# MundyRepo/MuNDy

Measured on AMD Instinct MI355X. Metric: timesteps/sec, 10^6 spherocylinders, frictionless LCP contact (BBPGD), higher is better.
Workload: dtype f64; 1 GPU; configs[2]: 1M spherocylinders r=0.5 L=2 at 40% volume fraction, random packing, AABB+0.1 neighbour list, frictionless LCP tol 1e-05; bodies_per_gpu=1000000, bodies_total=1000000, contacts_per_gpu=7621833, contacts_total=7621833, parallelism=single GPU (N > 1: the same system, hilbert domain decomposition with RCCL halo)

## Files before the change

mundy_amd/csrc/convex.hip:

```cpp
#include <cstdlib>
#include <memory>
#include <mutex>
#include <type_traits>
#include <vector>

#include "../../include/mundy_hip_contact_force.h"
#include "../../include/mundy_hip_hydro_solve.h"
#include "mhip_internal.hpp"

namespace mhip {

constexpr unsigned kProfileStride = 8;
constexpr double kSmallStep = 1e-6;
constexpr double kBBEps = 1e-15 * 10;
constexpr double kLowest = -1.7976931348623157e308;

#ifndef MHIP_STREAM_UNROLL
#define MHIP_STREAM_UNROLL 4
#endif
#ifndef MHIP_STREAM_GRID
#define MHIP_STREAM_GRID 1048576
#endif
constexpr int kStreamUnroll = MHIP_STREAM_UNROLL;
__device__ inline size_t stream_first() { return blockIdx.x * (size_t)(kBlock * kStreamUnroll) + threadIdx.x; }
// ... 314 lines not shown
  const unsigned g = stream_grid(vec ? (n + 1) / 2 : n);
  if (vec) k_copy<true><<<g, kBlock, 0, s>>>(n, dst, src);
  else k_copy<false><<<g, kBlock, 0, s>>>(n, dst, src);
  MHIP_LAUNCH_CHECK();
  return MHIP_SUCCESS;
}

#ifndef MHIP_NT
#define MHIP_NT 3
#endif
typedef double mhip_d2v __attribute__((ext_vector_type(2)));
typedef int mhip_i2v __attribute__((ext_vector_type(2)));
template <bool NT> __device__ inline double ld_s(const double* p) { return NT ? __builtin_nontemporal_load(p) : *p; }
template <bool NT> __device__ inline int32_t ld_s(const int32_t* p) { return NT ? __builtin_nontemporal_load(p) : *p; }
template <bool NT> __device__ inline double2 ld_s(const double2* p) {
  if (!NT) return *p;
  const mhip_d2v v = __builtin_nontemporal_load(reinterpret_cast<const mhip_d2v*>(p));
  return make_double2(v.x, v.y);
}
template <bool NT> __device__ inline int2 ld_s(const int2* p) {
  if (!NT) return *p;
  const mhip_i2v v = __builtin_nontemporal_load(reinterpret_cast<const mhip_i2v*>(p));
  return make_int2(v.x, v.y);
}
template <bool NT> __device__ inline V3 ld_s3(const double* p, size_t i) {
  return {ld_s<NT>(p + 3 * i), ld_s<NT>(p + 3 * i + 1), ld_s<NT>(p + 3 * i + 2)};
}

struct SolverState {
  double step, residual, num, den;
  unsigned iter;
  unsigned flips;
  int converged, done, converged_at_init;
};

enum XMode { X_APPLY = 0, X_INIT = 1, X_SOLVE = 2 };
enum Kinematics { KIN_TRANS = 0, KIN_RIGID = 1, KIN_ROD = 2 };

struct OpView {
  size_t C, N;
  const int2* pairs;
  const double *normal, *ra, *rb, *mt, *mr;
  const int32_t *inc_ptr, *inc;
  const double* half;
  double* vel;
  double dt;
  size_t body_first, body_count;
  const unsigned char* counted;
  const double *arc_s, *arc_t;
  const double* axis;
  double* omega;
  int xcd_aware;
  size_t c_first, c_end;
  unsigned part_offset, part_stride;
  unsigned long long* body_mask;
  const unsigned char* pos;
  const int32_t* aptr;
  const int32_t* aent;
  const double* arec;
  size_t arec_stride;
  const unsigned long long* snap_mask;
  double* vel_alt;
  double* drift;
  const double* arm_max;
  const double* fire_at;
  int32_t* fired;
  unsigned long long* tier_counters;
  double* force_rows;
};

__device__ inline size_t xcd_tile(size_t lin, size_t ntiles, unsigned T) {
  if (T == 0) return lin;
  const size_t W = 8 * (size_t)T;
  const size_t g = lin / W, r = lin % W;
  if ((g + 1) * W > ntiles) return lin;
  return g * W + (r % 8) * T + r / 8;
}

template <int MODE, bool PACKED, bool NT = false>
__device__ inline double2 iterate_load(size_t c, const double* __restrict__ xt, const double* __restrict__ gt) {
  if (MODE == X_SOLVE) {
    if (PACKED) return ld_s<NT>(reinterpret_cast<const double2*>(xt) + c);
    return make_double2(xt[c], gt[c]);
  }
  return make_double2(xt[c], 0.0);
}
template <int MODE>
__device__ inline double iterate_value(double2 p, double step, bool step_is_zero, const Space& sp) {
  if (MODE == X_SOLVE) {
    const double v = step_is_zero ? 1.0 * p.x : 1.0 * p.x + (-step) * p.y;
    return sp.project(v);
  }
  return p.x;
}
// ... 15 lines not shown
#ifndef MHIP_KBODY_FLAT
#define MHIP_KBODY_FLAT 2
#endif
#ifndef MHIP_KBODY_EARLY_FROM
#define MHIP_KBODY_EARLY_FROM 3
#endif
#ifndef MHIP_KBODY_FLAT3_ABOVE
#define MHIP_KBODY_FLAT3_ABOVE 0.9
#endif
template <int MODE, int KIN, int G, int U, bool PACKED, int TRACK = 0, int FLATP = 0>
__global__ void __launch_bounds__(kBlock, MHIP_KBODY_WAVES)
    k_body(OpView op, const SolverState* __restrict__ st, const double* __restrict__ X0, const double* __restrict__ X1,
           const double* __restrict__ G0, const double* __restrict__ G1, Space sp) {
  constexpr bool FLAT = FLATP > 0 && MODE == X_SOLVE && PACKED;
  constexpr bool kRegTrack = TRACK == 2 && MODE == X_SOLVE && PACKED;
  constexpr int kFlatPlanes = kRegTrack ? ((KIN == KIN_RIGID) ? 4 : 3) : ((KIN == KIN_RIGID) ? 3 : 2);
  __shared__ double2 flat_img[FLAT ? kFlatPlanes * FLATP * kBlock : 1];
  const size_t tile = xcd_tile(blockIdx.x, gridDim.x, op.xcd_aware);
  const size_t t = tile * (size_t)blockDim.x + threadIdx.x;
  const int sub = static_cast<int>(t % G);
  const bool has_body = t / G < op.body_count;
  if (!FLAT && !has_body) return;
  const size_t b = op.body_first + (has_body ? t / G : op.body_count - 1);
  int32_t E0 = 0, E1 = 0;
  if constexpr (FLAT) {
    if (op.aptr != nullptr) {
      const size_t tb0r = tile * (size_t)(kBlock / G);
      const size_t tb0 = (tb0r < op.body_count) ? tb0r : op.body_count;
      const size_t tb1 = (tb0 + kBlock / G < op.body_count) ? tb0 + kBlock / G : op.body_count;
      E0 = op.aptr[op.body_first + tb0];
      E1 = op.aptr[op.body_first + tb1];
    }
  }
  const double* xt = X0;
  const double* gt = G0;
  double step = 0.0;
  double* vel_new = op.vel;
  if (MODE == X_SOLVE) {
    const int done = st->done;
    const bool odd = st->flips & 1u;
    step = st->step;
    if (done) return;
    if (odd) {
      xt = X1;
      gt = G1;
    }
    if (op.vel_alt) vel_new = odd ? op.vel : op.vel_alt;
  }
  const bool step_is_zero = fabs(-step) < kZeroTol;
  constexpr int HW = (KIN == KIN_RIGID) ? 6 : (KIN == KIN_ROD ? 4 : 3);
  DD3 Fdd{{0.0, 0.0}, {0.0, 0.0}, {0.0, 0.0}}, Tdd{{0.0, 0.0}, {0.0, 0.0}, {0.0, 0.0}};
  const int32_t beg = op.inc_ptr[b], end = op.inc_ptr[b + 1];
  double mt = 0.0, mr = 0.0;
  V3 axis{0.0, 0.0, 0.0};
  constexpr bool track = TRACK != 0 && MODE == X_SOLVE && PACKED;
  constexpr bool track_regs = kRegTrack;
  constexpr bool track_rows = track && !track_regs;
  V3 dF{0.0, 0.0, 0.0}, dS{0.0, 0.0, 0.0};
  constexpr bool kEarlyTail = FLAT && FLATP >= MHIP_KBODY_EARLY_FROM && track;
  constexpr bool kEarlySnap = FLAT && FLATP >= MHIP_KBODY_EARLY_FROM;
  double drift_old = 0.0, fire_thr = 0.0;
  unsigned long long snap_early = 0ull;
  if (kEarlySnap) {
    const unsigned long long* src = (op.aptr != nullptr && op.body_mask != nullptr)
                                        ? op.snap_mask
                                        : reinterpret_cast<const unsigned long long*>(op.vel);
    snap_early = src[b];
  }
  unsigned long long mask_early = 0ull;
  if (kEarlySnap) {
    const unsigned long long* src = (op.body_mask != nullptr) ? op.body_mask
                                                              : reinterpret_cast<const unsigned long long*>(op.vel);
    mask_early = src[b];
  }
  double2 o0 = make_double2(0.0, 0.0), o1 = o0, o2 = o0;
  if (sub == 0) {
    mt = op.mt[b];
    if (KIN != KIN_TRANS) mr = op.mr[b];
    if (KIN == KIN_ROD) axis = load3(op.axis, b);
    if (kEarlyTail) {
      drift_old = op.drift[b];
      if (op.fire_at != nullptr) fire_thr = op.fire_at[b];
      if (track_rows) {
        const double* vel_old = op.vel_alt ? ((vel_new == op.vel) ? op.vel_alt : op.vel) : op.vel;
        const double2* vo = reinterpret_cast<const double2*>(vel_old + 6 * b);
        o0 = vo[0];
        o1 = vo[1];
        o2 = vo[2];
      }
    }
  }
  auto process = [&](const int32_t* __restrict__ ent, const double* __restrict__ rec, const int32_t* kk,
                     const bool eager, const size_t planes = 0) {
    int32_t e[U];
    double lam[U], xo[U];
    double2 h0[U], h1[U], h2[U];
    auto fetch = [&](int u) {
      const size_t k = static_cast<size_t>(kk[u]);
      if (planes != 0) {
        const double2* H2 = reinterpret_cast<const double2*>(rec) + k;
        h0[u] = H2[0];
        h1[u] = H2[planes];
        if (KIN == KIN_RIGID) h2[u] = H2[2 * planes];
      } else if (KIN == KIN_TRANS) {
        const double* H = rec + k * HW;
        h0[u] = make_double2(H[0], H[1]);
        h1[u] = make_double2(H[2], 0.0);
      } else {
        const double2* H2 = reinterpret_cast<const double2*>(rec + k * HW);
        h0[u] = H2[0];
        h1[u] = H2[1];
// ... 9 lines not shown
    double2 pit[U];
#pragma unroll
    for (int u = 0; u < U; ++u)
      pit[u] = iterate_load<MODE, PACKED>(e[u] >= 0 ? static_cast<size_t>(e[u] >> 1) : 0, xt, gt);
#pragma unroll
    for (int u = 0; u < U; ++u) {
      xo[u] = (track_regs && e[u] >= 0) ? pit[u].x : 0.0;
      lam[u] = (e[u] >= 0) ? iterate_value<MODE>(pit[u], step, step_is_zero, sp) : 0.0;
    }
    if (!eager) {
#pragma unroll
      for (int u = 0; u < U; ++u)
        if (lam[u] != 0.0 || (track_regs && xo[u] != 0.0)) fetch(u);
    }
#pragma unroll
    for (int u = 0; u < U; ++u) {
      if (lam[u] == 0.0 && !(track_regs && xo[u] != 0.0)) continue;
      const V3 n{h0[u].x, h0[u].y, h1[u].x};
      if (track_regs) {
        const double dl = (e[u] & 1) ? lam[u] - xo[u] : xo[u] - lam[u];
        const V3 df{dl * n.x, dl * n.y, dl * n.z};
        dF = dF + df;
        if (KIN == KIN_ROD) dS = dS + h1[u].y * df;
        if (KIN == KIN_RIGID) dS = dS + cross(V3{h1[u].y, h2[u].x, h2[u].y}, df);
      }
      if (lam[u] == 0.0) continue;
      V3 f{lam[u] * n.x, lam[u] * n.y, lam[u] * n.z};
      if (!(e[u] & 1)) f = V3{-f.x, -f.y, -f.z};
      dd_add(Fdd, f);
      if (KIN == KIN_RIGID) dd_add(Tdd, cross(V3{h1[u].y, h2[u].x, h2[u].y}, f));
      if (KIN == KIN_ROD) dd_add(Tdd, h1[u].y * f);
    }
  };
  const bool masked = PACKED && MODE == X_SOLVE && op.body_mask != nullptr && sp.kind == MHIP_SPACE_LOWER_BOUND &&
                      sp.lo == 0.0 && step >= 0.0 && step <= 1.7976931348623157e308;
  int32_t full_from = beg;
  if (masked) {
    if (op.aptr != nullptr) {
      const int32_t ab = op.aptr[b], ae = op.aptr[b + 1];
      if constexpr (FLAT) {
        constexpr int kChunk = FLATP * kBlock;
        constexpr bool NTS = (MHIP_NT & 1) != 0;
        double2* const pl0 = flat_img;
        double2* const pl1 = flat_img + kChunk;
        double2* const pl2 = flat_img + (kFlatPlanes - 1) * kChunk;
        for (int32_t base = E0; base < E1; base += kChunk) {
          int32_t fe[FLATP];
          double2 r0[FLATP], r1[FLATP], r2[FLATP];
          bool live[FLATP];
#pragma unroll
          for (int p = 0; p < FLATP; ++p) {
            const int32_t k = base + p * kBlock + static_cast<int32_t>(threadIdx.x);
            live[p] = k < E1;
            fe[p] = ld_s<NTS>(op.aent + (live[p] ? k : E1 - 1));
          }
#pragma unroll
          for (int p = 0; p < FLATP; ++p) {
            const int32_t k0 = base + p * kBlock + static_cast<int32_t>(threadIdx.x);
            const size_t k = static_cast<size_t>(live[p] ? k0 : E1 - 1);
            r2[p] = make_double2(0.0, 0.0);
            const double2* H2 = reinterpret_cast<const double2*>(op.arec) + k;
            r0[p] = ld_s<NTS>(H2);
            r1[p] = ld_s<NTS>(H2 + op.arec_stride);
            if (KIN == KIN_RIGID) r2[p] = ld_s<NTS>(H2 + 2 * op.arec_stride);
          }
#pragma unroll
          for (int p = 0; p < FLATP; ++p)
            if (!live[p]) fe[p] = -1;
          double2 pit[FLATP];
#pragma unroll
// ... 41 lines not shown
                if (a3.y != 0.0) {
                  const V3 df{a3.y * n.x, a3.y * n.y, a3.y * n.z};
                  dF = dF + df;
                  if (KIN == KIN_ROD) dS = dS + a1.y * df;
                  if (KIN == KIN_RIGID) dS = dS + cross(arm, df);
                }
                if (a3.x == 0.0) continue;
                const V3 fr{a3.x * n.x, a3.x * n.y, a3.x * n.z};
                dd_add(Fdd, fr);
                if (KIN == KIN_RIGID) dd_add(Tdd, cross(arm, fr));
                if (KIN == KIN_ROD) dd_add(Tdd, a1.y * fr);
                continue;
              }
              const V3 f{a0.x, a0.y, a1.x};
              dd_add(Fdd, f);
              if (KIN == KIN_RIGID) {
                const double2 a2 = pl2[slot];
                dd_add(Tdd, V3{a1.y, a2.x, a2.y});
              }
              if (KIN == KIN_ROD) dd_add(Tdd, a1.y * f);
            }
          }
          __syncthreads();
        }
      } else {
        for (int32_t k0 = ab + sub; k0 < ae; k0 += G * U) {
          int32_t kc[U];
#pragma unroll
          for (int u = 0; u < U; ++u) kc[u] = (k0 + u * G < ae) ? k0 + u * G : -1;
          process(op.aent, op.arec, kc, true, op.arec_stride);
        }
      }
    }
    const int32_t head = (end - beg < 64) ? end - beg : 64;
    unsigned long long mm = kEarlySnap ? mask_early : op.body_mask[b];
    if (head < 64) mm &= (1ull << head) - 1ull;
    if (op.aptr != nullptr) mm &= ~(kEarlySnap ? snap_early : op.snap_mask[b]);
    if (FLAT && !has_body) mm = 0ull;
    int32_t kk[U];
#pragma unroll
    for (int u = 0; u < U; ++u) kk[u] = -1;
    int rank = 0, nm = 0;
    while (mm) {
      const int bit = __ffsll(static_cast<long long>(mm)) - 1;
      mm &= mm - 1ull;
      if ((rank++ & (G - 1)) != sub) continue;
#pragma unroll
      for (int u = 0; u < U; ++u)
        if (nm == u) kk[u] = beg + bit;
      if (++nm == U) {
        process(op.inc, op.half, kk, true);
        nm = 0;
#pragma unroll
        for (int u = 0; u < U; ++u) kk[u] = -1;
      }
    }
    if (nm) process(op.inc, op.half, kk, true);
    full_from = beg + head;
  }
  if (FLAT && !has_body) return;
  for (int32_t k0 = full_from + sub; k0 < end; k0 += G * U) {
    int32_t kk[U];
#pragma unroll
    for (int u = 0; u < U; ++u) kk[u] = (k0 + u * G < end) ? k0 + u * G : -1;
    process(op.inc, op.half, kk, false);
  }
#pragma unroll
  for (int off = G / 2; off > 0; off >>= 1) {
    dd_add(Fdd.x, dd_shfl_xor(Fdd.x, off));
    dd_add(Fdd.y, dd_shfl_xor(Fdd.y, off));
    dd_add(Fdd.z, dd_shfl_xor(Fdd.z, off));
    if (KIN != KIN_TRANS) {
      dd_add(Tdd.x, dd_shfl_xor(Tdd.x, off));
      dd_add(Tdd.y, dd_shfl_xor(Tdd.y, off));
      dd_add(Tdd.z, dd_shfl_xor(Tdd.z, off));
    }
  }
  if (track_regs) {
#pragma unroll
    for (int off = G / 2; off > 0; off >>= 1) {
      dF = dF + V3{__shfl_xor(dF.x, off, 64), __shfl_xor(dF.y, off, 64), __shfl_xor(dF.z, off, 64)};
      if (KIN != KIN_TRANS) dS = dS + V3{__shfl_xor(dS.x, off, 64), __shfl_xor(dS.y, off, 64), __shfl_xor(dS.z, off, 64)};
    }
  }
  if (sub != 0) return;
  if (track_rows && !kEarlyTail) {
    const double* vel_old = op.vel_alt ? ((vel_new == op.vel) ? op.vel_alt : op.vel) : op.vel;
    const double2* vo = reinterpret_cast<const double2*>(vel_old + 6 * b);
    o0 = vo[0];
    o1 = vo[1];
    o2 = vo[2];
  }
  const V3 F = dd_value(Fdd), T = dd_value(Tdd);
  double2* v = reinterpret_cast<double2*>(vel_new + 6 * b);
  V3 W{0.0, 0.0, 0.0};
  if (KIN == KIN_RIGID) W = V3{mr * T.x, mr * T.y, mr * T.z};
  if (KIN == KIN_ROD) {
// ... 40 lines not shown
}

struct PointVelocities {
  V3 vi, vj;
};
template <int KIN>
__device__ inline PointVelocities contact_point_velocities(const OpView& op, const double* __restrict__ vel, size_t c,
                                                           int2 ij) {
  const double2* vi2 = reinterpret_cast<const double2*>(vel + 6 * (size_t)ij.x);
  const double2* vj2 = reinterpret_cast<const double2*>(vel + 6 * (size_t)ij.y);
  const double2 a0 = vi2[0], a1 = vi2[1], b0 = vj2[0], b1 = vj2[1];
  V3 vi{a0.x, a0.y, a1.x}, vj{b0.x, b0.y, b1.x};
  if (KIN == KIN_RIGID) {
    const double2 a2 = vi2[2], b2 = vj2[2];
    vi = vi + cross(V3{a1.y, a2.x, a2.y}, load3(op.ra, c));
    vj = vj + cross(V3{b1.y, b2.x, b2.y}, load3(op.rb, c));
  }
  if (KIN == KIN_ROD) {
    const double2 a2 = vi2[2], b2 = vj2[2];
    const double ci = rod_arm_coef(op.arc_s[c]), cj = rod_arm_coef(op.arc_t[c]);
    vi = vi + ci * V3{a1.y, a2.x, a2.y};
    vj = vj + cj * V3{b1.y, b2.x, b2.y};
  }
  return {vi, vj};
}
template <int KIN>
__device__ inline double contact_dt_sdot(const OpView& op, const double* __restrict__ vel, size_t c, int2 ij) {
  const V3 n = load3(op.normal, c);
  const auto [vi, vj] = contact_point_velocities<KIN>(op, vel, c, ij);
  const double sdot = -n.x * (vi.x - vj.x) - n.y * (vi.y - vj.y) - n.z * (vi.z - vj.z);
  return op.dt * sdot;
}

struct TierCheck {
  size_t H, I;
  double* wake;
  int32_t* list;
  unsigned long long* counters;
  const int32_t* fired;
  double* fire_at;
  unsigned blocks;
};

template <int KIN>
__device__ __forceinline__ void tier_evaluate(const OpView& op, const double* __restrict__ vel,
                                              const double* __restrict__ xt, double* __restrict__ xn,
                                              const double* __restrict__ q, const Space& sp, double step,
                                              bool step_is_zero, int resid_kind, size_t c, double& rmax, DD& num,
                                              DD& den) {
  const int2 ij = op.pairs[c];
  double x_old = 0.0, g_old = 0.0;
  const double xc = iterate_x<X_SOLVE, true>(c, xt, nullptr, step, step_is_zero, sp, &x_old, &g_old);
  const double y = contact_dt_sdot<KIN>(op, vel, c, ij);
  const double g = 1.0 * q[c] + 1.0 * y;
  reinterpret_cast<double2*>(xn)[c] = make_double2(xc, g);
  if (op.body_mask != nullptr && sp.kind == MHIP_SPACE_LOWER_BOUND && sp.lo == 0.0) {
    const bool was = !(x_old == 0.0 && g_old >= 0.0 && g_old <= 1.7976931348623157e308);
    const bool now = !(xc == 0.0 && g >= 0.0 && g <= 1.7976931348623157e308);
    if (was != now) {
      const unsigned pi = op.pos[2 * c], pj = op.pos[2 * c + 1];
      if (pi < 64u) atomicXor(&op.body_mask[ij.x], 1ull << pi);
      if (pj < 64u) atomicXor(&op.body_mask[ij.y], 1ull << pj);
    }
  }
  if (op.counted == nullptr || op.counted[c]) {
    const double r = residual_term(resid_kind, xc, g, sp);
    if (r > rmax) rmax = r;
    const double dx = xc - x_old;
    dd_add(num, dx * dx);
    dd_add(den, dx * (g - g_old));
  }
}

constexpr int kTierRoundClaims = 8;
constexpr int kTierQueue = kTierRoundClaims * kBlock;
template <int KIN>
__device__ __forceinline__ void tier_service(const OpView& op, const SolverState* __restrict__ st, double* __restrict__ X0,
                                             double* __restrict__ X1, const double* __restrict__ q, const Space& sp,
                                             int resid_kind, double* __restrict__ partials, const TierCheck& tc,
                                             unsigned block, size_t slot, double* scratch, int32_t* queue,
                                             unsigned* queued) {
  if (st->done) return;
  const double* xt = X0;
  double* xn = X1;
  if (st->flips & 1u) {
    xt = X1; xn = X0;
  }
  const double step = st->step;
  const double* vel = op.vel;
  if (op.vel_alt && !(st->flips & 1u)) vel = op.vel_alt;
  const bool step_is_zero = fabs(-step) < kZeroTol;
  double rmax = 0.0;
  DD num{0.0, 0.0}, den{0.0, 0.0};
  const size_t awake = static_cast<size_t>(tc.counters[2]);
  const size_t share = (awake + tc.blocks - 1) / tc.blocks;
// ... 114 lines not shown
    const double2 a0 = vi2[0], a1 = vi2[1], b0 = vj2[0], b1 = vj2[1];
    double2 a2 = make_double2(0.0, 0.0), b2 = make_double2(0.0, 0.0);
    if (KIN != KIN_TRANS) {
      a2 = vi2[2];
      b2 = vj2[2];
    }
    const double x_old = (MODE == X_SOLVE) ? pold.x : 0.0, g_old = (MODE == X_SOLVE) ? pold.y : 0.0;
    const double xc = iterate_value<MODE>(pold, step, step_is_zero, sp);
    V3 vi{a0.x, a0.y, a1.x}, vj{b0.x, b0.y, b1.x};
    if (KIN == KIN_RIGID) {
      vi = vi + cross(V3{a1.y, a2.x, a2.y}, arm_i);
      vj = vj + cross(V3{b1.y, b2.x, b2.y}, arm_j);
    }
    if (KIN == KIN_ROD) {
      const double ci = rod_arm_coef(arc_i), cj = rod_arm_coef(arc_j);
      vi = vi + ci * V3{a1.y, a2.x, a2.y};
      vj = vj + cj * V3{b1.y, b2.x, b2.y};
    }
    const double sdot = -n.x * (vi.x - vj.x) - n.y * (vi.y - vj.y) - n.z * (vi.z - vj.z);
    const double y = op.dt * sdot;
    if (MODE == X_APPLY) {
      gn[c] = y;
    } else {
      const double g = 1.0 * qc + 1.0 * y;
      if (PACKED) {
        reinterpret_cast<double2*>(xn)[c] = make_double2(xc, g);
        if (op.body_mask != nullptr && sp.kind == MHIP_SPACE_LOWER_BOUND && sp.lo == 0.0) {
          const bool was = (MODE == X_INIT) ? false : !(x_old == 0.0 && g_old >= 0.0 && g_old <= 1.7976931348623157e308);
          const bool now = !(xc == 0.0 && g >= 0.0 && g <= 1.7976931348623157e308);
          if (was != now) {
            const unsigned pi = op.pos[2 * c], pj = op.pos[2 * c + 1];
            if (pi < 64u) atomicXor(&op.body_mask[ij.x], 1ull << pi);
            if (pj < 64u) atomicXor(&op.body_mask[ij.y], 1ull << pj);
          }
        }
      } else {
        gn[c] = g;
        if (MODE == X_SOLVE) xn[c] = xc;
      }
      if (op.counted == nullptr || op.counted[c]) {
        const double r = residual_term(resid_kind, xc, g, sp);
        if (r > rmax) rmax = r;
        if (MODE == X_SOLVE) {
          const double dx = xc - x_old;
          dd_add(num, dx * dx);
          dd_add(den, dx * (g - g_old));
        }
      }
    }
  }
  if (MODE != X_APPLY) {
    const double m = block_max(rmax, scratch);
    const DD s1 = block_sum(num, scratch);
    const DD s2 = block_sum(den, scratch);
    if (threadIdx.x == 0) {
      const size_t stride = op.part_stride ? op.part_stride : nblk;
      store_partial(partials, stride, op.part_offset + bid, m, s1, s2);
    }
  }
}

constexpr int kFinalBlock = 1024;
template <class... Sums>
__device__ inline void reduce_records(int nparts, const double* __restrict__ partials, size_t si, size_t sk,
                                      double* scratch, double& rmax, Sums&... sums) {
  rmax = kLowest;
// ... 418 lines not shown

template <int KIN>
__global__ void __launch_bounds__(kBlock)
    k_half_build(size_t nent, const int32_t* __restrict__ inc, const double* __restrict__ normal,
                 const double* __restrict__ ra, const double* __restrict__ rb, const double* __restrict__ arc_s,
                 const double* __restrict__ arc_t, double* __restrict__ half) {
  constexpr int HW = (KIN == KIN_RIGID) ? 6 : (KIN == KIN_ROD ? 4 : 3);
  for (size_t k = blockIdx.x * (size_t)blockDim.x + threadIdx.x; k < nent; k += (size_t)gridDim.x * blockDim.x) {
    const int32_t e = inc[k];
    const size_t c = static_cast<size_t>(e >> 1);
    double* H = half + k * HW;
    const V3 n = load3(normal, c);
    H[0] = n.x; H[1] = n.y; H[2] = n.z;
    if (KIN == KIN_RIGID) {
      const V3 r = (e & 1) ? load3(rb, c) : load3(ra, c);
      H[3] = r.x; H[4] = r.y; H[5] = r.z;
    }
    if (KIN == KIN_ROD) H[3] = rod_arm_coef((e & 1) ? arc_t[c] : arc_s[c]);
  }
}

__global__ void __launch_bounds__(kBlock) k_pos_build(size_t N, const int32_t* __restrict__ inc_ptr,
                                                     const int32_t* __restrict__ inc, unsigned char* __restrict__ pos) {
  for (size_t b = blockIdx.x * (size_t)blockDim.x + threadIdx.x; b < N; b += (size_t)gridDim.x * blockDim.x) {
    const int32_t beg = inc_ptr[b], end = inc_ptr[b + 1];
    for (int32_t k = beg; k < end; ++k) {
      const int32_t e = inc[k];
      const int32_t slot = k - beg;
      pos[2 * static_cast<size_t>(e >> 1) + (e & 1)] = static_cast<unsigned char>(slot < 255 ? slot : 255);
    }
  }
}
__global__ void __launch_bounds__(kBlock)
    k_active_count(size_t first, size_t count, const int32_t* __restrict__ inc_ptr,
                   const unsigned long long* __restrict__ body_mask, int32_t* __restrict__ cnt) {
  for (size_t t = blockIdx.x * (size_t)blockDim.x + threadIdx.x; t < count; t += (size_t)gridDim.x * blockDim.x) {
    const size_t b = first + t;
    const int32_t deg = inc_ptr[b + 1] - inc_ptr[b];
    unsigned long long m = body_mask[b];
    if (deg < 64) m &= (1ull << deg) - 1ull;
    cnt[t] = __popcll(m);
  }
}
template <int HW>
__global__ void __launch_bounds__(kBlock)
    k_active_fill_flat(size_t first, size_t count, const int32_t* __restrict__ inc_ptr, const int32_t* __restrict__ inc,
                       const double* __restrict__ half, const unsigned long long* __restrict__ body_mask,
                       const int32_t* __restrict__ aptr_local, int32_t* __restrict__ aptr, int32_t* __restrict__ aent,
                       double* __restrict__ arec, size_t stride, unsigned long long* __restrict__ snap_mask) {
  __shared__ unsigned long long tmask[kBlock];
  __shared__ int32_t tbeg[kBlock];
  __shared__ int32_t tptr[kBlock + 1];
  const size_t t0 = blockIdx.x * (size_t)kBlock;
  if (t0 >= count) return;
  const int nb = static_cast<int>(count - t0 < (size_t)kBlock ? count - t0 : (size_t)kBlock);
  const int tid = static_cast<int>(threadIdx.x);
  if (tid < nb) {
    const size_t t = t0 + tid, b = first + t;
    const int32_t beg = inc_ptr[b], deg = inc_ptr[b + 1] - beg;
    unsigned long long m = body_mask[b];
    if (deg < 64) m &= (1ull << deg) - 1ull;
    snap_mask[b] = m;
    const int32_t out = aptr_local[t];
    aptr[b] = out;
    if (t + 1 == count) aptr[b + 1] = aptr_local[count];
    tmask[tid] = m;
    tbeg[tid] = beg;
    tptr[tid] = out;
  }
  if (tid == 0) tptr[nb] = aptr_local[t0 + nb];
  __syncthreads();
  const int32_t E0 = tptr[0], E1 = tptr[nb];
  for (int32_t o = E0 + tid; o < E1; o += kBlock) {
    int lo = 0, hi = nb;
    while (hi - lo > 1) {
      const int mid = (lo + hi) >> 1;
      if (tptr[mid] <= o) lo = mid; else hi = mid;
    }
    unsigned long long m = tmask[lo];
    for (int r = o - tptr[lo]; r > 0; --r) m &= m - 1ull;
    const size_t k = static_cast<size_t>(tbeg[lo] + (__ffsll(static_cast<long long>(m)) - 1));
    aent[o] = inc[k];
    double2* dst = reinterpret_cast<double2*>(arec) + o;
    if (HW % 2 == 0) {
      const double2* src = reinterpret_cast<const double2*>(half + k * HW);
#pragma unroll
      for (int w = 0; w < HW / 2; ++w) dst[w * stride] = src[w];
    } else {
      const double* src = half + k * HW;
      dst[0] = make_double2(src[0], src[1]);
      dst[stride] = make_double2(src[2], 0.0);
    }
  }
}

__global__ void __launch_bounds__(kBlock) k_rod_axes(size_t n, const double* __restrict__ seg, double* __restrict__ axis) {
  for (size_t i = blockIdx.x * (size_t)blockDim.x + threadIdx.x; i < n; i += (size_t)gridDim.x * blockDim.x) {
    const double* r = seg + 8 * i;
    store3(axis, i, V3{r[3], r[4], r[5]} - V3{r[0], r[1], r[2]});
  }
}
__global__ void __launch_bounds__(kBlock) k_rate_rows(size_t n, const double* __restrict__ vel,
                                                     const double* __restrict__ axis, double* __restrict__ out) {
// ... 417 lines not shown
    store3(g, c, s.g);
  }
}

}

using namespace mhip;

struct ProfilingEvents {
  std::vector<hipEvent_t> v;
  ProfilingEvents() = default;
  ProfilingEvents(ProfilingEvents&& o) noexcept : v(std::move(o.v)) { o.v.clear(); }
  ProfilingEvents& operator=(ProfilingEvents&& o) noexcept {
    if (this != &o) {
      destroy();
      v = std::move(o.v);
      o.v.clear();
    }
    return *this;
  }
  ~ProfilingEvents() { destroy(); }
  void destroy() {
    for (auto ev : v) (void)hipEventDestroy(ev);
    v.clear();
  }
};
struct OpWorkspaces {
  HandleBuffer inc_ptr, inc, cursor, vel, partials, state, scanws, half, axis, omega, vel_out;
  HandleBuffer force_rows;
  HandleBuffer iterate;
  HandleBuffer rate_rows;
  HandleBuffer body_mask, pos;
  HandleBuffer sort_tmp, sort_list;
  HandleBuffer aptr, aent, arec, snap_mask, acnt;
  HandleBuffer tier_geo[2], tier_iter[2], tier_misc, tier_vel2, tier_drift, tier_arm, tier_xprev;
  PinnedBlock<SolverState> host_state;
  ProfilingEvents events;
  int device = -1;
};
static_assert(std::is_nothrow_move_constructible_v<OpWorkspaces> && std::is_nothrow_move_assignable_v<OpWorkspaces> &&
                  !std::is_copy_constructible_v<OpWorkspaces>,
              "the workspace set is handed over whole");

struct mhip_contact_op : OpWorkspaces {
  OpView view{};
  bool rot = false;
  int kin = KIN_TRANS;
  hipStream_t last_stream = nullptr;
  int tiering = 1;
  int drift_source = 0;
  int lanes_per_body = 2;
  struct Stage {
    const double* q = nullptr;
    double *x = nullptr, *g = nullptr, *x_tmp = nullptr, *g_tmp = nullptr;
    Space sp{0, 0, 0};
    mhip_pgd_config cfg{0, 0, 0};
    bool active = false;
    unsigned part_used = 0;
    double *P0 = nullptr, *P1 = nullptr;
    const double* q_cur = nullptr;
    size_t interior = 0;
    bool interior_known = false, pause_on_bad_step = false;
    unsigned polls = 0, iter_at_poll = 0, snap_at = 0;
  } stage;
  struct Tier {
    bool active = false;
    bool tracking = false;
// ... 98 lines not shown
#define MHIP_FOLD_ABOVE 4096
#endif
#ifndef MHIP_FOLD_BLOCK
#define MHIP_FOLD_BLOCK 128
#endif
inline void fold_partials(unsigned& nparts, size_t& stride, double*& parts, const SolverState* st, int check_done,
                          hipStream_t s) {
  if (nparts <= MHIP_FOLD_ABOVE) return;
  double* folded = parts + kRed * stride;
  k_fold_partials<<<kFoldGroups, kBlock, 0, s>>>((int)nparts, stride, parts, st, check_done, folded);
  parts = folded;
  nparts = kFoldGroups;
  stride = kFoldGroups;
}
inline unsigned final_block(size_t n) { return n <= 256 ? 64u : (n <= 2048 ? 256u : (unsigned)kFinalBlock); }
constexpr unsigned kStageStride = 2 * 32768;
constexpr int kMaxConstraintGrid = 32768;
unsigned constraint_grid(size_t C) {
  const size_t g = (C + kBlock - 1) / kBlock;
  return static_cast<unsigned>(g == 0 ? 1 : (g > (size_t)kMaxConstraintGrid ? kMaxConstraintGrid : g));
}

int op_snapshot_active(mhip_contact_op* op, hipStream_t s) {
  OpView& v = op->view;
  if (v.body_mask == nullptr || v.C == 0 || v.body_count == 0) return MHIP_SUCCESS;
  const size_t N = v.N, C = v.C, cnt = v.body_count;
  const int hw = (op->kin == KIN_RIGID) ? 6 : (op->kin == KIN_ROD ? 4 : 3);
  if (int e = op->aptr.reserve((N + 2) * sizeof(int32_t))) return e;
  if (int e = op->acnt.reserve((N + 2) * sizeof(int32_t))) return e;
  if (int e = op->aent.reserve((2 * C + 2) * sizeof(int32_t))) return e;
  const size_t stride = 2 * C + 2;
  if (int e = op->arec.reserve(stride * ((hw + 1) / 2) * sizeof(double2))) return e;
  if (int e = op->snap_mask.reserve((N + 2) * sizeof(unsigned long long))) return e;
  int32_t* local = op->cursor.as<int32_t>();
  k_active_count<<<grid_for(cnt), kBlock, 0, s>>>(v.body_first, cnt, v.inc_ptr, v.body_mask, op->acnt.as<int32_t>());
  MHIP_LAUNCH_CHECK();
  if (int e = exclusive_scan_i32(op->acnt.as<int32_t>(), local, cnt, op->scanws.ptr, s)) return e;
  pick<6, 4, 3>(hw, [&](auto h) {
    k_active_fill_flat<decltype(h)::value><<<grid_exact(cnt), kBlock, 0, s>>>(
        v.body_first, cnt, v.inc_ptr, v.inc, v.half, v.body_mask, local, op->aptr.as<int32_t>(), op->aent.as<int32_t>(),
        op->arec.as<double>(), stride, op->snap_mask.as<unsigned long long>());
  });
  MHIP_LAUNCH_CHECK();
  if (op->host_state != nullptr)
    MHIP_HIP(hipMemcpyAsync(reinterpret_cast<int32_t*>(op->host_state + 1), op->aptr.as<int32_t>() + v.body_first + cnt,
                            sizeof(int32_t), hipMemcpyDeviceToHost, s));
  v.aptr = op->aptr.as<int32_t>();
  v.aent = op->aent.as<int32_t>();
  v.arec = op->arec.as<double>();
  v.arec_stride = stride;
  v.snap_mask = op->snap_mask.as<unsigned long long>();
  return MHIP_SUCCESS;
}
constexpr unsigned kSnapshotAfter = 8;

constexpr double kTierMinGap = 1e-9;
constexpr size_t kTierMinContacts = 1500000;
#ifndef MHIP_TIER_RETIER_PERCENT
#define MHIP_TIER_RETIER_PERCENT 4
#endif
constexpr unsigned kTierHorizon = 64;
#ifndef MHIP_TIER_SHARE
#define MHIP_TIER_SHARE 0.45
#endif
constexpr double kTierShare = MHIP_TIER_SHARE;
#ifndef MHIP_TIER_SERVICE_BLOCKS
#define MHIP_TIER_SERVICE_BLOCKS 32
#endif
constexpr unsigned kTierFireBlocks = MHIP_TIER_SERVICE_BLOCKS;

struct TierGeo {
  int2* pairs;
  double *normal, *arc_s, *arc_t, *q, *ra, *rb;
  int32_t* orig;
  unsigned char* pos;
};
inline size_t tier_align(size_t b) { return (b + 255) & ~static_cast<size_t>(255); }
inline size_t tier_geo_bytes(size_t C, bool arms) {
  return tier_align(C * 8) + tier_align(3 * C * 8) + 3 * tier_align(C * 8) + tier_align(C * 4) + tier_align(2 * C) +
         (arms ? 2 * tier_align(3 * C * 8) : 0) + 256;
}
inline TierGeo tier_geo_at(void* base, size_t C) {
  char* p = static_cast<char*>(base);
  TierGeo g;
// ... 1024 lines not shown
    return MHIP_SUCCESS;
  }
  *velocity = op->view.vel;
  return MHIP_SUCCESS;
}

int mhip_bbpgd_solve_contact(mhip_contact_op_t op, const double* q, const mhip_space* space,
                             const mhip_pgd_config* config, double* x, double* g, double* x_tmp, double* g_tmp,
                             mhip_solve_result* result, mhip_stream_t stream) {
  TraceRange trace_range("solve_cqpp (fused BBPGD)");
  MHIP_REQUIRE(op != nullptr && result != nullptr, MHIP_ERR_INVALID_ARGUMENT, "null handle / result");
  if (int e = check_config(config)) return e;
  Space sp;
  if (int e = to_space(space, &sp)) return e;
  const size_t C = op->view.C;
  hipStream_t s = as_stream(stream);
  if (C == 0) {
    result->num_iters = 0;
    result->residual = config->residual_kind == MHIP_RESIDUAL_PROJECTED_DIFF ? kLowest / kSmallStep : kLowest;
    result->converged = 1;
    return MHIP_SUCCESS;
  }
  MHIP_REQUIRE(q && x && g && x_tmp && g_tmp, MHIP_ERR_INVALID_ARGUMENT, "solver vectors must not be null");
  MHIP_REQUIRE(x != x_tmp && g != g_tmp && x != g, MHIP_ERR_INVALID_ARGUMENT, "solver vectors must not alias");
  SolverState* st = op->state.as<SolverState>();
  double* parts = op->partials.as<double>();
  const unsigned cgrid = constraint_grid(C);
  const int rk = config->residual_kind;
  if (int e = op->iterate.reserve(2 * (C + 1) * sizeof(double2))) return e;
  double* P0 = op->iterate.as<double>();
  double* P1 = P0 + 2 * C;
  if (op->view.body_mask) MHIP_HIP(hipMemsetAsync(op->view.body_mask, 0x00, op->view.N * sizeof(unsigned long long), s));
  op->view.aptr = nullptr;
  if (int e = op_launch_body(op, X_INIT, x, x, nullptr, nullptr, sp, s)) return e;
  if (int e = op_launch_constraint(op, X_INIT, P0, P1, x, nullptr, q, sp, rk, cgrid, s, true)) return e;
  finalize_sweep<X_INIT>(op, cgrid, config, s);
  MHIP_LAUNCH_CHECK();
  unsigned enqueued = 0, chunk = 8, last_todo = 0, iter_before = 0;
  const bool prof = op->profile;
  if (prof && op->events.v.empty()) {
    op->events.v.resize(3 * 64);
    for (auto& ev : op->events.v) MHIP_HIP(hipEventCreate(&ev));
  }
  mhip_contact_op::Tier& tier = op->tier;
  tier.disabled = !tier_eligible(op, sp, rk) || op->tiering == 0;
  tier.tiered_iterations = tier.retiers = tier.wakeups = 0;
  tier.hot_sum = 0.0;
  TierPairs cur{P0, P1, q};
  struct TierGuard {
    mhip_contact_op* op;
    ~TierGuard() {
      if (!op->tier.active) {
        op->view.vel_alt = nullptr;
        op->view.drift = nullptr;
        op->tier.tracking = false;
        return;
      }
      op->tier.tracking = false;
      const size_t C2 = op->view.C;
      const TierGeo geo = tier_geo_at(op->tier_geo[op->tier.set].ptr, C2);
      k_tier_remap_inc<<<grid_for(2 * C2), kBlock, 0, op->last_stream>>>(2 * C2, op->inc.as<int32_t>(), geo.orig);
      (void)hipStreamSynchronize(op->last_stream);
      const int xa = op->view.xcd_aware;
      op->view = op->tier.saved;
      op->view.xcd_aware = xa;
      op->view.aptr = nullptr;
      op->tier.active = false;
    }
  } tier_guard{op};
  PollPlan plan;
  for (;;) {
    MHIP_HIP(hipMemcpyAsync(op->host_state, st, sizeof(SolverState), hipMemcpyDeviceToHost, s));
    MHIP_HIP(hipStreamSynchronize(s));
    if (prof && last_todo) {
      unsigned eff = op->host_state->iter - iter_before + ((op->host_state->converged && op->host_state->iter < config->max_iters) ? 1u : 0u);
      if (eff > last_todo) eff = last_todo;
      for (unsigned k = 0; k < eff; k += kProfileStride) {
        float a = 0.f, b = 0.f;
        MHIP_HIP(hipEventElapsedTime(&a, op->events.v[3 * k], op->events.v[3 * k + 1]));
        MHIP_HIP(hipEventElapsedTime(&b, op->events.v[3 * k + 1], op->events.v[3 * k + 2]));
        op->body_ms += a;
        op->constraint_ms += b;
        op->timed_iterations += 1;
      }
    }
    if (tier.active && last_todo) {
      unsigned ran = op->host_state->iter - iter_before + ((op->host_state->converged && op->host_state->iter < config->max_iters) ? 1u : 0u);
      if (ran > last_todo) ran = last_todo;
      tier.tiered_iterations += ran;
      tier.hot_sum += ran * (static_cast<double>(tier.H) / static_cast<double>(C));
    }
    if (op->host_state->done == 2) {
      if (int e = tier_release(op, cur, false, P0, P1, q, nullptr, nullptr, nullptr, nullptr, s)) return e;
      tier.disabled = true;
      op->host_state->done = 0;
      MHIP_HIP(hipMemcpyAsync(&st->done, &op->host_state->done, sizeof(int), hipMemcpyHostToDevice, s));
      enqueued = op->host_state->iter;
    }
    if (op->host_state->done || enqueued >= config->max_iters) break;
    if (enqueued == 0)
      if (int e = op_snapshot_active(op, s)) return e;
    const bool light = plan.light_poll();
    if (!light) {
      const size_t retiers_before = tier.retiers;
      if (!tier.disabled && (enqueued >= kSnapshotAfter || !tier.tracking)) {
        const unsigned left = config->max_iters - enqueued;
        if (int e = tier_update(op, cur, op->host_state->iter, left < chunk ? left : chunk, C, true, s)) return e;
      }
      if (enqueued >= kSnapshotAfter)
        if (int e = op_snapshot_active(op, s)) return e;
      plan.full_poll_done(enqueued, *reinterpret_cast<const int32_t*>(op->host_state + 1),
                          tier.retiers != retiers_before, !tier.disabled && !tier.active);
    }
    iter_before = op->host_state->iter;
    const unsigned stretch = plan.stretch(chunk, op->host_state->iter, op->host_state->residual, config->tol, C);
    const unsigned todo = (config->max_iters - enqueued < stretch) ? config->max_iters - enqueued : stretch;
#ifdef MHIP_TIER_DEBUG
    fprintf(stderr, "poll: iter %u residual %.3e light %d quiet %u stretch %u (regular %u) snapshot entries %d\n",
            op->host_state->iter, op->host_state->residual, (int)light, plan.quiet, stretch, chunk,
            *reinterpret_cast<const int32_t*>(op->host_state + 1));
#endif
    for (unsigned k = 0; k < todo; ++k) {
      const bool pk = prof && (k % kProfileStride == 0);
      if (pk) MHIP_HIP(hipEventRecord(op->events.v[3 * k], s));
      if (int e = op_launch_body(op, X_SOLVE, cur.P0, cur.P1, nullptr, nullptr, sp, s, true)) return e;
      if (pk) MHIP_HIP(hipEventRecord(op->events.v[3 * k + 1], s));
      unsigned np = cgrid;
      size_t ps = cgrid;
      if (tier.active) {
        if (int e = op_launch_constraint_tiered(op, cur, sp, rk, &np, s)) return e;
        ps = kStageStride;
      } else {
        if (int e = op_launch_constraint(op, X_SOLVE, cur.P0, cur.P1, nullptr, nullptr, q, sp, rk, cgrid, s, true)) return e;
      }
// ... 664 lines not shown
```

Measured before the change: 8.796 timesteps/s.

## Skip per-body incidence and mask loads for clean waves and uniform mobilities

Adds a per-wave dirty byte array, built when the active snapshot is taken and set whenever a contact's mask bit flips. Wavefronts whose bodies have no mask changes and no long incidence lists skip loading inc_ptr, snap and body masks and the head mask walk. It also adds a kernel that detects uniform translational and rotational mobilities so the body kernel can read a scalar instead of per-body arrays. The cost is extra state and dirty-marking stores in the constraint kernels, plus correctness risk if the dirty tracking misses an update.

```diff
diff --git a/mundy_amd/csrc/convex.hip b/mundy_amd/csrc/convex.hip
--- a/mundy_amd/csrc/convex.hip
+++ b/mundy_amd/csrc/convex.hip
@@ -370,6 +370,8 @@
   unsigned iter;
   unsigned flips;
   int converged, done, converged_at_init;
+  int mt_mixed, mr_mixed;
+  double mt_one, mr_one;
 };
 
 enum XMode { X_APPLY = 0, X_INIT = 1, X_SOLVE = 2 };
@@ -398,6 +400,9 @@
   const double* arec;
   size_t arec_stride;
   const unsigned long long* snap_mask;
+  unsigned char* wave_dirty;
+  int mob_uniform;
+  double mt_one, mr_one;
   double* vel_alt;
   double* drift;
   const double* arm_max;
@@ -479,6 +484,12 @@
       E1 = op.aptr[op.body_first + tb1];
     }
   }
+  constexpr bool kCleanWaves = FLAT && G == 2;
+  static_assert(kBlock == 256, "a tile's clean-wave bytes are read as one 32-bit word");
+  unsigned dirty_word = ~0u;
+  if constexpr (kCleanWaves) {
+    if (op.aptr != nullptr && op.wave_dirty != nullptr) dirty_word = reinterpret_cast<const unsigned*>(op.wave_dirty)[tile];
+  }
   const double* xt = X0;
   const double* gt = G0;
   double step = 0.0;
@@ -497,7 +508,21 @@
   const bool step_is_zero = fabs(-step) < kZeroTol;
   constexpr int HW = (KIN == KIN_RIGID) ? 6 : (KIN == KIN_ROD ? 4 : 3);
   DD3 Fdd{{0.0, 0.0}, {0.0, 0.0}, {0.0, 0.0}}, Tdd{{0.0, 0.0}, {0.0, 0.0}, {0.0, 0.0}};
-  const int32_t beg = op.inc_ptr[b], end = op.inc_ptr[b + 1];
+  const bool masked = PACKED && MODE == X_SOLVE && op.body_mask != nullptr && sp.kind == MHIP_SPACE_LOWER_BOUND &&
+                      sp.lo == 0.0 && step >= 0.0 && step <= 1.7976931348623157e308;
+  bool clean = false;
+  if constexpr (kCleanWaves) {
+    const unsigned wave = static_cast<unsigned>(__builtin_amdgcn_readfirstlane(static_cast<int>(threadIdx.x >> 6)));
+    clean = masked && ((dirty_word >> (8u * wave)) & 0xffu) == 0u;
+  }
+  struct {
+    int32_t beg, end;
+    unsigned long long snap_early, mask_early;
+  } own;
+  if (!clean) {
+    own.beg = op.inc_ptr[b];
+    own.end = op.inc_ptr[b + 1];
+  }
   double mt = 0.0, mr = 0.0;
   V3 axis{0.0, 0.0, 0.0};
   constexpr bool track = TRACK != 0 && MODE == X_SOLVE && PACKED;
@@ -507,23 +532,24 @@
   constexpr bool kEarlyTail = FLAT && FLATP >= MHIP_KBODY_EARLY_FROM && track;
   constexpr bool kEarlySnap = FLAT && FLATP >= MHIP_KBODY_EARLY_FROM;
   double drift_old = 0.0, fire_thr = 0.0;
-  unsigned long long snap_early = 0ull;
-  if (kEarlySnap) {
+  if (kEarlySnap && !clean) {
     const unsigned long long* src = (op.aptr != nullptr && op.body_mask != nullptr)
                                         ? op.snap_mask
                                         : reinterpret_cast<const unsigned long long*>(op.vel);
-    snap_early = src[b];
-  }
-  unsigned long long mask_early = 0ull;
-  if (kEarlySnap) {
+    own.snap_early = src[b];
+  }
+  if (kEarlySnap && !clean) {
     const unsigned long long* src = (op.body_mask != nullptr) ? op.body_mask
                                                               : reinterpret_cast<const unsigned long long*>(op.vel);
-    mask_early = src[b];
+    own.mask_early = src[b];
   }
   double2 o0 = make_double2(0.0, 0.0), o1 = o0, o2 = o0;
   if (sub == 0) {
-    mt = op.mt[b];
-    if (KIN != KIN_TRANS) mr = op.mr[b];
+    mt = op.mt_one;
+    mr = op.mr_one;
+    if (!(op.mob_uniform & 1)) mt = op.mt[b];
+    if (KIN != KIN_TRANS && !(op.mob_uniform & 2)) mr = op.mr[b];
+    if (KIN == KIN_TRANS) mr = 0.0;
     if (KIN == KIN_ROD) axis = load3(op.axis, b);
     if (kEarlyTail) {
       drift_old = op.drift[b];
@@ -599,10 +625,11 @@
       if (KIN == KIN_ROD) dd_add(Tdd, h1[u].y * f);
     }
   };
-  const bool masked = PACKED && MODE == X_SOLVE && op.body_mask != nullptr && sp.kind == MHIP_SPACE_LOWER_BOUND &&
-                      sp.lo == 0.0 && step >= 0.0 && step <= 1.7976931348623157e308;
-  int32_t full_from = beg;
-  if (masked) {
+  int32_t full_from = 0, full_end = 0;
+  if (!masked) {
+    full_from = own.beg;
+    full_end = own.end;
+  } else {
     if (op.aptr != nullptr) {
       const int32_t ab = op.aptr[b], ae = op.aptr[b + 1];
       if constexpr (FLAT) {
@@ -710,37 +737,49 @@
         }
       }
     }
-    const int32_t head = (end - beg < 64) ? end - beg : 64;
-    unsigned long long mm = kEarlySnap ? mask_early : op.body_mask[b];
-    if (head < 64) mm &= (1ull << head) - 1ull;
-    if (op.aptr != nullptr) mm &= ~(kEarlySnap ? snap_early : op.snap_mask[b]);
-    if (FLAT && !has_body) mm = 0ull;
+    if (!clean) {
+      const int32_t beg = own.beg, end = own.end;
+      const int32_t head = (end - beg < 64) ? end - beg : 64;
+      unsigned long long mm, snap = 0ull;
+      if (kEarlySnap) {
+        mm = own.mask_early;
+        snap = own.snap_early;
+        asm volatile("" : "+v"(snap));
+      } else {
+        mm = op.body_mask[b];
+        if (op.aptr != nullptr) snap = op.snap_mask[b];
+      }
+      if (head < 64) mm &= (1ull << head) - 1ull;
+      if (op.aptr != nullptr) mm &= ~snap;
+      if (FLAT && !has_body) mm = 0ull;
+      int32_t kk[U];
+#pragma unroll
+      for (int u = 0; u < U; ++u) kk[u] = -1;
+      int rank = 0, nm = 0;
+      while (mm) {
+        const int bit = __ffsll(static_cast<long long>(mm)) - 1;
+        mm &= mm - 1ull;
+        if ((rank++ & (G - 1)) != sub) continue;
+#pragma unroll
+        for (int u = 0; u < U; ++u)
+          if (nm == u) kk[u] = beg + bit;
+        if (++nm == U) {
+          process(op.inc, op.half, kk, true);
+          nm = 0;
+#pragma unroll
+          for (int u = 0; u < U; ++u) kk[u] = -1;
+        }
+      }
+      if (nm) process(op.inc, op.half, kk, true);
+      full_from = beg + head;
+      full_end = end;
+    }
+  }
+  if (FLAT && !has_body) return;
+  for (int32_t k0 = full_from + sub; k0 < full_end; k0 += G * U) {
     int32_t kk[U];
 #pragma unroll
-    for (int u = 0; u < U; ++u) kk[u] = -1;
-    int rank = 0, nm = 0;
-    while (mm) {
-      const int bit = __ffsll(static_cast<long long>(mm)) - 1;
-      mm &= mm - 1ull;
-      if ((rank++ & (G - 1)) != sub) continue;
-#pragma unroll
-      for (int u = 0; u < U; ++u)
-        if (nm == u) kk[u] = beg + bit;
-      if (++nm == U) {
-        process(op.inc, op.half, kk, true);
-        nm = 0;
-#pragma unroll
-        for (int u = 0; u < U; ++u) kk[u] = -1;
-      }
-    }
-    if (nm) process(op.inc, op.half, kk, true);
-    full_from = beg + head;
-  }
-  if (FLAT && !has_body) return;
-  for (int32_t k0 = full_from + sub; k0 < end; k0 += G * U) {
-    int32_t kk[U];
-#pragma unroll
-    for (int u = 0; u < U; ++u) kk[u] = (k0 + u * G < end) ? k0 + u * G : -1;
+    for (int u = 0; u < U; ++u) kk[u] = (k0 + u * G < full_end) ? k0 + u * G : -1;
     process(op.inc, op.half, kk, false);
   }
 #pragma unroll
@@ -847,6 +886,11 @@
   return op.dt * sdot;
 }
 
+__device__ inline void mark_wave_dirty(const OpView& op, int32_t body) {
+  const size_t rel = static_cast<size_t>(body) - op.body_first;
+  if (rel < op.body_count) op.wave_dirty[rel >> 5] = 1;
+}
+
 struct TierCheck {
   size_t H, I;
   double* wake;
@@ -876,6 +920,10 @@
       const unsigned pi = op.pos[2 * c], pj = op.pos[2 * c + 1];
       if (pi < 64u) atomicXor(&op.body_mask[ij.x], 1ull << pi);
       if (pj < 64u) atomicXor(&op.body_mask[ij.y], 1ull << pj);
+      if (now && op.wave_dirty != nullptr) {
+        if (pi < 64u) mark_wave_dirty(op, ij.x);
+        if (pj < 64u) mark_wave_dirty(op, ij.y);
+      }
     }
   }
   if (op.counted == nullptr || op.counted[c]) {
@@ -1056,6 +1104,10 @@
             const unsigned pi = op.pos[2 * c], pj = op.pos[2 * c + 1];
             if (pi < 64u) atomicXor(&op.body_mask[ij.x], 1ull << pi);
             if (pj < 64u) atomicXor(&op.body_mask[ij.y], 1ull << pj);
+            if (MODE == X_SOLVE && now && op.wave_dirty != nullptr) {
+              if (pi < 64u) mark_wave_dirty(op, ij.x);
+              if (pj < 64u) mark_wave_dirty(op, ij.y);
+            }
           }
         }
       } else {
@@ -1540,6 +1592,23 @@
   }
 }
 __global__ void __launch_bounds__(kBlock)
+    k_mob_uniform(size_t first, size_t count, const double* __restrict__ mt, const double* __restrict__ mr,
+                  SolverState* __restrict__ st) {
+  const long long t0 = __double_as_longlong(mt[first]);
+  const long long r0 = mr != nullptr ? __double_as_longlong(mr[first]) : 0ll;
+  bool tm = false, rm = false;
+  for (size_t t = blockIdx.x * (size_t)blockDim.x + threadIdx.x; t < count; t += (size_t)gridDim.x * blockDim.x) {
+    tm = tm || __double_as_longlong(mt[first + t]) != t0;
+    if (mr != nullptr) rm = rm || __double_as_longlong(mr[first + t]) != r0;
+  }
+  if (tm) st->mt_mixed = 1;
+  if (rm) st->mr_mixed = 1;
+  if (blockIdx.x == 0 && threadIdx.x == 0) {
+    st->mt_one = __longlong_as_double(t0);
+    st->mr_one = __longlong_as_double(r0);
+  }
+}
+__global__ void __launch_bounds__(kBlock)
     k_active_count(size_t first, size_t count, const int32_t* __restrict__ inc_ptr,
                    const unsigned long long* __restrict__ body_mask, int32_t* __restrict__ cnt) {
   for (size_t t = blockIdx.x * (size_t)blockDim.x + threadIdx.x; t < count; t += (size_t)gridDim.x * blockDim.x) {
@@ -1555,7 +1624,8 @@
     k_active_fill_flat(size_t first, size_t count, const int32_t* __restrict__ inc_ptr, const int32_t* __restrict__ inc,
                        const double* __restrict__ half, const unsigned long long* __restrict__ body_mask,
                        const int32_t* __restrict__ aptr_local, int32_t* __restrict__ aptr, int32_t* __restrict__ aent,
-                       double* __restrict__ arec, size_t stride, unsigned long long* __restrict__ snap_mask) {
+                       double* __restrict__ arec, size_t stride, unsigned long long* __restrict__ snap_mask,
+                       unsigned char* __restrict__ wave_dirty) {
   __shared__ unsigned long long tmask[kBlock];
   __shared__ int32_t tbeg[kBlock];
   __shared__ int32_t tptr[kBlock + 1];
@@ -1563,9 +1633,11 @@
   if (t0 >= count) return;
   const int nb = static_cast<int>(count - t0 < (size_t)kBlock ? count - t0 : (size_t)kBlock);
   const int tid = static_cast<int>(threadIdx.x);
+  bool long_list = false;
   if (tid < nb) {
     const size_t t = t0 + tid, b = first + t;
     const int32_t beg = inc_ptr[b], deg = inc_ptr[b + 1] - beg;
+    long_list = deg > 64;
     unsigned long long m = body_mask[b];
     if (deg < 64) m &= (1ull << deg) - 1ull;
     snap_mask[b] = m;
@@ -1577,6 +1649,8 @@
     tptr[tid] = out;
   }
   if (tid == 0) tptr[nb] = aptr_local[t0 + nb];
+  const unsigned long long longs = __ballot(long_list);
+  if ((tid & 31) == 0 && tid < nb) wave_dirty[(t0 + tid) >> 5] = ((longs >> (tid & 32)) & 0xffffffffull) != 0ull;
   __syncthreads();
   const int32_t E0 = tptr[0], E1 = tptr[nb];
   for (int32_t o = E0 + tid; o < E1; o += kBlock) {
@@ -2060,7 +2134,7 @@
   HandleBuffer rate_rows;
   HandleBuffer body_mask, pos;
   HandleBuffer sort_tmp, sort_list;
-  HandleBuffer aptr, aent, arec, snap_mask, acnt;
+  HandleBuffer aptr, aent, arec, snap_mask, acnt, wave_dirty;
   HandleBuffer tier_geo[2], tier_iter[2], tier_misc, tier_vel2, tier_drift, tier_arm, tier_xprev;
   PinnedBlock<SolverState> host_state;
   ProfilingEvents events;
@@ -2225,6 +2299,12 @@
   const size_t stride = 2 * C + 2;
   if (int e = op->arec.reserve(stride * ((hw + 1) / 2) * sizeof(double2))) return e;
   if (int e = op->snap_mask.reserve((N + 2) * sizeof(unsigned long long))) return e;
+  {
+    const void* const before = op->wave_dirty.ptr;
+    const size_t bytes = ((N + 127) / 128 + 8) * sizeof(unsigned);
+    if (int e = op->wave_dirty.reserve(bytes)) return e;
+    if (op->wave_dirty.ptr != before) MHIP_HIP(hipMemsetAsync(op->wave_dirty.ptr, 0, bytes, s));
+  }
   int32_t* local = op->cursor.as<int32_t>();
   k_active_count<<<grid_for(cnt), kBlock, 0, s>>>(v.body_first, cnt, v.inc_ptr, v.body_mask, op->acnt.as<int32_t>());
   MHIP_LAUNCH_CHECK();
@@ -2232,7 +2312,7 @@
   pick<6, 4, 3>(hw, [&](auto h) {
     k_active_fill_flat<decltype(h)::value><<<grid_exact(cnt), kBlock, 0, s>>>(
         v.body_first, cnt, v.inc_ptr, v.inc, v.half, v.body_mask, local, op->aptr.as<int32_t>(), op->aent.as<int32_t>(),
-        op->arec.as<double>(), stride, op->snap_mask.as<unsigned long long>());
+        op->arec.as<double>(), stride, op->snap_mask.as<unsigned long long>(), op->wave_dirty.as<unsigned char>());
   });
   MHIP_LAUNCH_CHECK();
   if (op->host_state != nullptr)
@@ -2243,6 +2323,7 @@
   v.arec = op->arec.as<double>();
   v.arec_stride = stride;
   v.snap_mask = op->snap_mask.as<unsigned long long>();
+  v.wave_dirty = op->wave_dirty.as<unsigned char>();
   return MHIP_SUCCESS;
 }
 constexpr unsigned kSnapshotAfter = 8;
@@ -3333,6 +3414,13 @@
   double* P1 = P0 + 2 * C;
   if (op->view.body_mask) MHIP_HIP(hipMemsetAsync(op->view.body_mask, 0x00, op->view.N * sizeof(unsigned long long), s));
   op->view.aptr = nullptr;
+  op->view.mob_uniform = 0;
+  if (op->view.body_count > 0) {
+    MHIP_HIP(hipMemsetAsync(&st->mt_mixed, 0, 2 * sizeof(int), s));
+    k_mob_uniform<<<grid_for(op->view.body_count), kBlock, 0, s>>>(op->view.body_first, op->view.body_count, op->view.mt,
+                                                                  op->kin != KIN_TRANS ? op->view.mr : nullptr, st);
+    MHIP_LAUNCH_CHECK();
+  }
   if (int e = op_launch_body(op, X_INIT, x, x, nullptr, nullptr, sp, s)) return e;
   if (int e = op_launch_constraint(op, X_INIT, P0, P1, x, nullptr, q, sp, rk, cgrid, s, true)) return e;
   finalize_sweep<X_INIT>(op, cgrid, config, s);
@@ -3351,6 +3439,10 @@
   struct TierGuard {
     mhip_contact_op* op;
     ~TierGuard() {
+      struct ForgetMobilities {
+        mhip_contact_op* op;
+        ~ForgetMobilities() { op->view.mob_uniform = 0; }
+      } forget{op};
       if (!op->tier.active) {
         op->view.vel_alt = nullptr;
         op->view.drift = nullptr;
@@ -3399,8 +3491,15 @@
       enqueued = op->host_state->iter;
     }
     if (op->host_state->done || enqueued >= config->max_iters) break;
-    if (enqueued == 0)
+    if (enqueued == 0) {
       if (int e = op_snapshot_active(op, s)) return e;
+      if (op->view.body_count > 0) {
+        const SolverState& hs = *op->host_state;
+        op->view.mob_uniform = (hs.mt_mixed ? 0 : 1) | ((op->kin != KIN_TRANS && !hs.mr_mixed) ? 2 : 0);
+        op->view.mt_one = hs.mt_one;
+        op->view.mr_one = hs.mr_one;
+      }
+    }
     const bool light = plan.light_poll();
     if (!light) {
       const size_t retiers_before = tier.retiers;
```

Measured after the change: 8.984 timesteps/s (median of 6 runs). 2.1% higher.
